# jjfiv/fastrank

Hardware: AMD Instinct MI355X
Metric: coordinate-ascent NDCG@10 evals/sec on MSLR-WEB30K shape (higher is better)
Workload: dtype f64; 1 GPU; synthetic MSLR-WEB30K shape: 3800000 docs x 136 features x 31000 queries, coordinate ascent NDCG@10, 32 restarts/GPU x 25 steps/coord (configs[2]); restarts_total=32, parallelism=restart-sharded x1 (dataset replicated), launcher=single process

## Files before the change

fastrank_amd/clib.py:

```python
import ctypes as C
import json
import os
from typing import Dict, List, Optional, Set

from . import _build

_MODEL_TYPES = ["SingleFeature", "Linear", "DecisionTree", "Ensemble"]


ALLREDUCE_SUM_FN = C.CFUNCTYPE(C.c_int, C.c_void_p, C.POINTER(C.c_double), C.c_size_t)


class _CResult(C.Structure):
    _fields_ = [("error_message", C.c_void_p), ("success", C.c_void_p)]


_lib = None


def _load():
    global _lib
    if _lib is not None:
        return _lib
    path = _build.LIB_PATH
    if _build.needs_build():
        try:
            _build.build()
        except Exception as exc:
            if not os.path.exists(path):
                raise ImportError(
                    "libfastrank_amd.so is not built and could not be built: {}".format(exc)
                ) from exc
    L = C.CDLL(path)
    vp, sz = C.c_void_p, C.c_size_t
    res = C.POINTER(_CResult)
    sigs = {
        "free_str": (None, [vp]),
        "free_c_result": (None, [res]),
        "free_dataset": (None, [vp]),
        "free_model": (None, [vp]),
        "free_cqrel": (None, [vp]),
        "load_cqrel": (res, [C.c_char_p]),
        "cqrel_from_json": (res, [C.c_char_p]),
        "cqrel_query_json": (vp, [vp, C.c_char_p]),
        "load_ranksvm_format": (res, [C.c_char_p, C.c_char_p]),
        "dataset_query_sampling": (res, [vp, C.c_char_p]),
        "dataset_feature_sampling": (res, [vp, C.c_char_p]),
        "dataset_query_json": (vp, [vp, C.c_char_p]),
        "query_json": (vp, [C.c_char_p]),
        "make_dense_dataset_f32_f64_i64": (res, [sz, sz, vp, vp, vp]),
        "train_model": (res, [C.c_char_p, vp]),
        "model_from_json": (res, [C.c_char_p]),
        "model_query_json": (vp, [vp, C.c_char_p]),
        "evaluate_by_query": (vp, [vp, vp, vp, C.c_char_p]),
        "predict_scores": (vp, [vp, vp]),
        "predict_to_trecrun": (vp, [vp, vp, C.c_char_p, C.c_char_p, sz]),
        "fr_device_count": (C.c_int, []),
        "fr_set_device": (C.c_int, [C.c_int]),
        "fr_version": (C.c_char_p, []),
        "fr_train_model_shard": (vp, [C.c_char_p, vp, C.c_uint32, C.c_uint32]),
        "fr_select_model": (res, [C.c_char_p, C.c_int]),
        "fr_ca_begin": (vp, [C.c_char_p, vp, C.c_uint32, C.c_uint32, C.POINTER(vp)]),
        "fr_ca_begin_query_shard": (vp, [C.c_char_p, vp, C.c_uint64, ALLREDUCE_SUM_FN, vp, C.POINTER(vp)]),
        "fr_ca_step": (vp, [vp, C.c_uint64, C.POINTER(C.c_uint64), C.POINTER(C.c_int)]),
        "fr_ca_state": (vp, [vp]),
        "fr_ca_free": (None, [vp]),
        "fr_last_train_stats": (vp, []),
        "fr_predict_scores_dense": (vp, [vp, vp, vp, sz]),
        "fr_debug_lambda_gradients": (vp, [vp, vp, vp, C.c_char_p, C.c_double, vp, vp, sz]),
        "fr_debug_hist_bins": (vp, [vp, C.c_uint32, sz, sz, vp, vp, vp, vp, vp]),
        "fr_debug_hist_tree": (res, [vp, C.c_uint32, C.c_uint32, C.c_uint32, vp, vp, sz]),
        "fr_debug_lambdamart_sample": (vp, [vp, C.c_char_p, C.c_uint32]),
        "fr_debug_lambda_gradients_sampled": (vp, [vp, vp, vp, C.c_char_p, C.c_double, vp, sz, vp, vp, sz]),
        "fr_debug_hist_tree_sampled": (res, [vp, C.c_uint32, C.c_uint32, C.c_uint32, vp, vp, sz, vp, sz, vp, sz]),
        "fr_evaluate_dense": (vp, [vp, vp, vp, C.c_char_p, vp, sz, C.POINTER(vp)]),
        "fr_rank_order": (vp, [vp, vp, vp, sz, vp, sz]),
        "fr_dataset_num_queries": (sz, [vp]),
        "fr_dataset_num_instances": (sz, [vp]),
        "fr_dataset_device_info": (vp, [vp]),
        "fr_evaluate_candidates": (vp, [vp, vp, C.c_char_p, sz, vp, vp, vp, vp, vp, vp]),
        "fr_profile_enable": (None, [C.c_int]),
        "fr_profile_reset": (None, []),
        "fr_profile_json": (vp, []),
        "fr_debug_resident_bound": (C.c_double, [C.c_int, C.c_double, C.c_double, C.c_double]),
        "fr_synchronize": (C.c_int, []),
        "fr_debug_device_plan": (vp, [C.c_char_p, C.c_int, C.c_uint32, C.c_int]),
        "fr_debug_fullrank_class": (C.c_uint32, [C.c_uint32]),
        "fr_debug_restart_queue": (vp, [C.c_uint32, C.c_uint32, C.c_uint32, vp, C.c_uint32]),
        "fr_dataset_release_replicas": (sz, [vp]),
        "fr_debug_peer_copy": (vp, [C.c_int, C.c_int, sz]),
        "fr_pack_restart_records": (vp, [C.c_char_p, sz, sz, vp]),
        "fr_unpack_restart_records": (vp, [vp, sz, sz]),
        "fr_rccl_allgather": (vp, [vp, sz, vp, sz, vp]),
        "fr_debug_rccl_selftest": (vp, [C.c_int]),
        "fr_debug_walk_tiles": (vp, [vp, vp, vp, sz, vp, vp, sz, sz]),
    }
    for name, (restype, argtypes) in sigs.items():
        fn = getattr(L, name)
        fn.restype = restype
        fn.argtypes = argtypes
    _lib = L
    return L


EXPORTED_SYMBOLS = None


def exported_symbols() -> List[str]:
    _load()
    return [
        "free_str", "free_c_result", "free_dataset", "free_model", "free_cqrel", "load_cqrel",
        "cqrel_from_json", "cqrel_query_json", "load_ranksvm_format", "dataset_query_sampling",
        "dataset_feature_sampling", "dataset_query_json", "query_json",
        "make_dense_dataset_f32_f64_i64", "train_model", "model_from_json", "model_query_json",
        "evaluate_by_query", "predict_scores", "predict_to_trecrun",
    ]


def _take_str(ptr) -> Optional[str]:
    if not ptr:
        return None
    try:
        return C.cast(ptr, C.c_char_p).value.decode("utf-8")
    finally:
        _load().free_str(ptr)


def _raise_if_error_str(text: Optional[str]):
    if text is None:
        return
    if "{" in text:
        payload = json.loads(text)
        if "error" in payload and "context" in payload:
            raise Exception("{0}: {1}".format(payload["error"], payload["context"]))
    else:
        raise Exception(text)


def _raise_if_error_json(payload):
    if isinstance(payload, dict) and "error" in payload and "context" in payload:
        raise Exception("{0}: {1}".format(payload["error"], payload["context"]))


def _unwrap(result_ptr):
    if not result_ptr:
        raise ValueError("CResult should not be NULL")
    res = result_ptr.contents
    err_ptr, ok_ptr = res.error_message, res.success
    _load().free_c_result(result_ptr)
    _raise_if_error_str(_take_str(err_ptr))
    return ok_ptr


def _status(ptr):
    _raise_if_error_str(_take_str(ptr))


def _json_reply(ptr):
    payload = json.loads(_take_str(ptr))
    _raise_if_error_json(payload)
    return payload


class CQRel:

    def __init__(self, pointer=None):
        self.pointer = pointer
        self._queries = None

    def __del__(self):
        if getattr(self, "pointer", None) is not None and _lib is not None:
            _lib.free_cqrel(self.pointer)
            self.pointer = None

    @staticmethod
    def load_file(path: str) -> "CQRel":
        return CQRel(_unwrap(_load().load_cqrel(path.encode("utf-8"))))

# ... 207 lines not shown
```

fastrank_amd/csrc/capi.cpp:

```cpp
#include <atomic>
#include <limits>
#include <chrono>
#include <cstdio>
#include <cstdlib>
#include <cstring>
#include <fstream>

#include "../../include/fastrank.h"
#include "host.hpp"
#include "loader.hpp"
#include "lambdamart.hpp"
#include "rf_train.hpp"

using fr::FrError;
using frjson::Value;

struct CDataset {
    std::shared_ptr<fr::DatasetView> view;
};
struct CModel {
    fr::Model actual;
};
struct CQRel {
    fr::QRel actual;
// ... 961 lines not shown

const void* fr_debug_peer_copy(int src_device, int dst_device, size_t bytes) {
    return json_call([&]() {
        int can = 0, en = 0;
        double ms = 0.0;
        std::string err;
        if (!frdev::peer_copy_probe(src_device, dst_device, bytes, &can, &en, &ms, &err)) fr::fail_str(err);
        Value o = Value::object();
        o.set("src", Value::uint((uint64_t)src_device));
        o.set("dst", Value::uint((uint64_t)dst_device));
        o.set("bytes", Value::uint((uint64_t)bytes));
        o.set("can_access", Value::boolean(can != 0));
        o.set("enabled", Value::boolean(en != 0));
        o.set("ms", Value::number(ms));
        o.set("gbps", Value::number(ms > 0.0 ? (double)bytes / (ms * 1e-3) / 1e9 : 0.0));
        return frjson::dump(o);
    });
}

static std::vector<fr::RestartResult> restarts_from_json_text(const std::string& text) {
    Value v = parse_json_or_fail(text);
    if (!v.is_array()) fr::fail_raw("Error(\"invalid type: expected a sequence\", line: 1, column: 1)");
    std::vector<fr::RestartResult> hist;
    for (const auto& r : v.arr) {
        fr::RestartResult h;
        h.restart_id = (uint32_t)fr::json_u64(fr::json_field(r, "restart_id"), "restart_id");
        h.score = fr::json_f64(fr::json_field(r, "score"), "score");
        for (const auto& x : fr::json_field(r, "weights").arr) h.weights.push_back(fr::json_f64(x, "weights"));
        hist.push_back(std::move(h));
    }
    return hist;
}

const void* fr_pack_restart_records(const void* restarts_json, size_t cap, size_t dim, double* out) {
    return status_call([&]() {
        if (out == nullptr) fr::fail_str("fr_pack_restart_records: null output buffer");
        fr::pack_restart_records(restarts_from_json_text(accept_str("restarts_json", restarts_json)), cap, dim, out);
    });
}

const void* fr_unpack_restart_records(const double* records, size_t n_records, size_t dim) {
    return json_call([&]() {
        if (records == nullptr && n_records > 0) fr::fail_str("fr_unpack_restart_records: null input buffer");
        return frjson::dump(restarts_to_json(fr::unpack_restart_records(records, n_records, dim)));
    });
}

const void* fr_rccl_allgather(const int* devices, size_t n, const double* blocks, size_t block_len, double* out) {
    return json_call([&]() {
        if ((devices == nullptr || blocks == nullptr) && n > 0) fr::fail_str("fr_rccl_allgather: null argument");
        std::vector<int> devs(devices, devices + n);
        frdev::RcclReport rep;
        std::vector<double> got;
        std::string err;
        if (!frdev::rccl_allgather(devs, blocks, block_len, &got, &rep, &err)) fr::fail_str(err);
        if (rep.ran && out != nullptr) std::memcpy(out, got.data(), got.size() * sizeof(double));
        return frjson::dump(rccl_report_to_json(rep));
    });
}

const void* fr_debug_walk_tiles(const uint32_t* run_pos, const uint32_t* run_q0, const uint32_t* run_q1, size_t nruns, const uint32_t* qstart,
                                const uint32_t* qlen, size_t nq, size_t np) {
    return json_call([&]() {
        if (nruns > 0 && (!run_pos || !run_q0 || !run_q1)) fr::fail_str("fr_debug_walk_tiles: null run table");
        if (nq > 0 && (!qstart || !qlen)) fr::fail_str("fr_debug_walk_tiles: null query table");
        for (size_t q = 0; q < nq; q++)
            if ((size_t)qstart[q] + qlen[q] > np) fr::fail_str("fr_debug_walk_tiles: a query lies beyond np");
        for (size_t r = 0; r < nruns; r++)
            if (run_q0[r] > run_q1[r] || run_q1[r] > nq) fr::fail_str("fr_debug_walk_tiles: a run names queries that do not exist");
        const frdev::WalkTileLayout wl = frdev::build_walk_tiles(std::vector<uint32_t>(run_pos, run_pos + nruns), std::vector<uint32_t>(run_q0, run_q0 + nruns),
                                                                std::vector<uint32_t>(run_q1, run_q1 + nruns), std::vector<uint32_t>(qstart, qstart + nq),
                                                                std::vector<uint32_t>(qlen, qlen + nq), np);
        Value o = Value::object();
        auto list = [](const auto& v) {
            Value a = Value::array();
            for (auto x : v) a.push(Value::uint((uint64_t)x));
            return a;
        };
        o.set("walk_tile", Value::uint(frdev::WALK_TILE));
        o.set("wt_start", list(wl.wt_start));
        o.set("run_wt0", list(wl.run_wt0));
        o.set("seg", list(wl.seg));
        o.set("wofs", list(wl.wofs));
        return frjson::dump(o);
    });
}

const void* fr_debug_rccl_selftest(int device) {
    return json_call([&]() {
        std::vector<double> block(16), got;
        for (size_t i = 0; i < block.size(); i++) block[i] = 0.5 + (double)i;
        frdev::RcclReport rep;
        std::string err;
        if (!frdev::rccl_allgather(std::vector<int>(1, device), block.data(), block.size(), &got, &rep, &err, 1)) fr::fail_str(err);
        return frjson::dump(rccl_report_to_json(rep));
    });
}

int fr_set_device(int ordinal) {
    std::string err;
    if (!frdev::set_device(ordinal, &err)) return 1;
    frdev::warm_device(ordinal);
    g_pinned_device = ordinal;
    return 0;
}

const char* fr_version(void) { return "fastrank_amd 0.1.0 (fastrank C ABI 0.9.0-dev / python 0.7.0)"; }

const void* fr_train_model_shard(const void* train_request_json, const CDataset* dataset, uint32_t restart_begin,
                                 uint32_t restart_end) {
    return json_call([&]() {
        const CDataset& ds = require_dataset(dataset);
        ParsedRequest rq = parse_train_request(accept_str("train_request_json", train_request_json));
        if (rq.learner != Learner::CoordinateAscent) fr::fail_str("fr_train_model_shard: only CoordinateAscent shards by restart");
        std::lock_guard<std::mutex> lk(api_mu_of(ds));
        std::vector<fr::RestartResult> hist;
        train_ca(ds.view, rq, restart_begin, restart_end, &hist);
        Value o = Value::object();
        o.set("restarts", restarts_to_json(hist));
        {
            std::lock_guard<std::mutex> slk(g_stats_mu);
            o.set("stats", stats_to_json(g_last_stats));
        }
        return frjson::dump(o);
    });
}

struct FrTrainer {
    std::unique_ptr<fr::CATrainer> t;
    std::chrono::steady_clock::time_point t0;
    std::shared_ptr<fr::DataCore> core;
};

void* fr_ca_begin(const void* train_request_json, const CDataset* dataset, uint32_t restart_begin,
                  uint32_t restart_end, const void** error_out) {
    if (error_out) *error_out = nullptr;
    FrTrainer* h = nullptr;
    const void* st = status_call([&]() {
        const CDataset& ds = require_dataset(dataset);
        ParsedRequest rq = parse_train_request(accept_str("train_request_json", train_request_json));
        if (rq.learner != Learner::CoordinateAscent) fr::fail_str("fr_ca_begin: only CoordinateAscent");
        std::lock_guard<std::mutex> lk(api_mu_of(ds));
        fr::Evaluator ev = fr::make_evaluator(*ds.view, rq.measure, rq.has_qrel ? &rq.qrel : nullptr);
        if (ds.view->host_csr().nq == 0) fr::fail_str("assertion failed: !data.queries().is_empty()");
        auto holder = std::make_unique<FrTrainer>();
        holder->t0 = std::chrono::steady_clock::now();
        holder->t = std::make_unique<fr::CATrainer>(ds.view, std::move(ev), rq.ca, restart_begin, restart_end);
        holder->core = ds.view->core;
        h = holder.release();
    });
    if (st) {
        if (error_out) *error_out = st; else free((void*)st);
        return nullptr;
    }
    return h;
}

void* fr_ca_begin_query_shard(const void* train_request_json, const CDataset* dataset, uint64_t total_queries,
                              fr_allreduce_sum_fn allreduce, void* ctx, const void** error_out) {
    if (error_out) *error_out = nullptr;
    FrTrainer* h = nullptr;
    const void* st = status_call([&]() {
        const CDataset& ds = require_dataset(dataset);
        ParsedRequest rq = parse_train_request(accept_str("train_request_json", train_request_json));
        if (rq.learner != Learner::CoordinateAscent) fr::fail_str("fr_ca_begin_query_shard: only CoordinateAscent");
        if (!allreduce) fr::fail_str("fr_ca_begin_query_shard: allreduce callback is null!");
// ... 458 lines not shown
```

fastrank_amd/csrc/device.hpp:

```cpp
#pragma once
#include <algorithm>
#include <cstddef>
#include <cstdint>
#include <memory>
#include <string>
#include <vector>

namespace frdev {

const char* path_env(const char* name);
inline const char* pricing_env(const char* name) {
#ifdef FR_PRICING
    return path_env(name);
#else
    (void)name;
    return nullptr;
#endif
}

enum Measure : int { M_NDCG = 0, M_AP = 1, M_RR = 2 };

constexpr uint32_t WALK_TILE = 128;
struct WalkTileLayout {
    std::vector<uint32_t> wt_start, run_wt0;
// ... 134 lines not shown
        unsigned long long pairs = 0, redone = 0;
    };
    bool linesearch_submit(int ctx, int measure, int64_t depth, const double* norms, const std::vector<LineGroup>& groups,
                           std::string* err);
    bool linesearch_collect(int ctx, std::vector<double>* means, LsCounts* counts, std::string* err);
    bool linesearch(int measure, int64_t depth, const double* norms, const std::vector<LineGroup>& groups,
                    std::vector<double>* means, LsCounts* counts, std::string* err);
    uint64_t resident_reserve(size_t slots, std::string* err);
    bool resident_store_from_scores(uint64_t owner, size_t slot, size_t b, std::string* err);
    const std::vector<double>& column_absmax() const;
    unsigned long long exact_fallbacks() const;
    void routing_counters(unsigned long long* exact_groups, unsigned long long* redo_entries) const;
    void chain_counters(unsigned long long* runs, unsigned long long* visits, unsigned long long* ranked_on = nullptr,
                        unsigned long long* ranked_off = nullptr) const;
    void audit_counters(unsigned long long* values, unsigned long long* mismatches) const;
    bool download_last_matrix(std::vector<double>* out, size_t* ldm, std::string* err);

    struct RfActive { uint32_t tree, key, n; };
    struct RfCand { double position, importance; uint32_t ids_i, flags, pos_l, pos_r; double sum_l, sum_r; };
    struct RfSplit { int32_t fslot; uint32_t pos, left, right; };
    bool rf_set_presence(const uint32_t* bits_by_instance, size_t words, size_t n_instances, std::string* err);
    bool rf_begin(const std::vector<uint32_t>& root_off, const std::vector<uint32_t>& root_ids, uint32_t nf,
                  const std::vector<uint32_t>& feats, std::string* err, const uint32_t* positions = nullptr,
                  bool lambda_targets = false);
    bool rf_positions(const std::vector<uint32_t>& root_ids, uint32_t* positions , std::string* err);
    bool rf_root_outputs(std::vector<double>* out, std::string* err);
    bool rf_level(const std::vector<RfActive>& active, const std::vector<uint32_t>& slot_of_key, uint32_t k, int method,
                  uint32_t min_leaf, std::vector<RfCand>* cands, std::vector<float>* label_minmax, std::string* err);
    bool rf_split(const std::vector<RfSplit>& splits, std::vector<double>* child_out, std::string* err);
    void rf_end();
    size_t rf_bytes_per_item() const { return 41; }

    bool lambda_gradients(const double* norms, int64_t depth, double sigma, std::string* err, const unsigned char* query_flags = nullptr);
    bool lambda_download_positions(std::vector<double>* lambda, std::vector<double>* weight, std::string* err);
    bool lambda_download(double* lambda_by_instance, double* weight_by_instance, size_t out_len, std::string* err,
                         const unsigned char* query_flags = nullptr);

    struct HistNode { uint32_t slot, begin, end; };
    struct HistSplit { uint32_t begin, end, fslot, edge, nl; };
    struct HistSub { uint32_t parent, small, large; };
    struct HistBest { double imp; long long ql, qtot; uint32_t edge, nl, valid, pad; };
    bool hist_bins(const uint32_t* positions, size_t n, const std::vector<uint32_t>& feats, uint32_t k, bool* built, std::string* err);
    bool hist_edges(std::vector<float>* edges, std::vector<uint32_t>* nedges, std::string* err);
    bool hist_download_bins(uint8_t* out , size_t len, std::string* err);
    bool hist_sample(const unsigned char* query_flags, uint32_t n_t, const uint32_t* fsel, size_t f_t, std::string* err);
    bool hist_quantise(const double* lam_list, const double* wt_list, int* s_l, int* s_w, bool* all_zero, std::string* err);
    bool hist_root(std::string* err);
    bool hist_search(const std::vector<HistNode>& nodes, uint32_t min_leaf, std::vector<HistBest>* best, std::string* err);
    bool hist_split(const std::vector<HistSplit>& splits, const std::vector<HistNode>& builds, const std::vector<HistSub>& subs,
                    uint32_t next_slots, std::string* err);
    bool hist_leaf_sums(const std::vector<HistNode>& leaves, std::vector<long long>* qw , std::string* err);
    void hist_end();

    int take_flags();

  private:
    DeviceDataset();
    bool try_score_trees_rank(const FlatTrees& trees, std::string* err);
    bool try_score_trees_lds(const FlatTrees& trees, std::string* err);
    bool try_score_trees_lds_shape(const FlatTrees& trees, const void* shape, std::string* err);
    struct Impl;
    Impl* impl_;
};

int device_count(std::string* err);
bool set_device(int ordinal, std::string* err);
void warm_device(int ordinal);
void profile_enable(bool on);
void profile_reset();
std::vector<KernelStat> profile_stats();
bool device_synchronize(std::string* err);
struct RcclReport {
    bool ran = false, matches_host_gather = false;
    int ranks = 0;
    std::vector<int> devices;
    size_t block_doubles = 0;
    double init_us = 0.0, first_us = 0.0, us = 0.0;
    std::string reason;
    std::string library;
};
bool rccl_allgather(const std::vector<int>& devices, const double* blocks, size_t block_len, std::vector<double>* gathered, RcclReport* rep,
                    std::string* err, size_t min_ranks = 2);
bool peer_copy_probe(int src, int dst, size_t bytes, int* can_access, int* enabled, double* ms, std::string* err);
size_t device_free_bytes();
void* pinned_alloc(size_t bytes);
void pinned_free(void* p);
void fullrank_class_of(uint32_t len, uint32_t* nl, uint32_t* pl);

}
```

fastrank_amd/csrc/kernels_order.inc:

```
constexpr uint32_t WT = WALK_TILE;
constexpr uint32_t WT_DPL = WT / 64;

__device__ __forceinline__ void order_segment(uint32_t s, uint32_t idx, uint32_t len, uint32_t* lo, uint32_t* hi) {
    *lo = s & 0xFFu;
    *hi = s >> 8;
    if (idx >= len || *hi <= *lo) {
        *lo = idx;
        *hi = idx + 1u;
    }
}

constexpr int ORDER_OQ = 2;
__global__ __launch_bounds__(WAVE) void xslot_kernel(const float4* __restrict__ xb, const uint16_t* __restrict__ seg, const uint32_t* __restrict__ wt_start,
                                                     uint32_t np, uint32_t dq, uint32_t d, uint8_t* __restrict__ out) {
    __shared__ float4 xs[ORDER_OQ][WT];
    const uint32_t lane = threadIdx.x;
    const uint32_t pb = wt_start[blockIdx.x];
    const uint32_t len = min(wt_start[blockIdx.x + 1] - pb, WT);
    const uint32_t j0 = blockIdx.y * ORDER_OQ;
    uint32_t lo[WT_DPL], hi[WT_DPL];
    float4 mine[WT_DPL][ORDER_OQ];
#pragma unroll
    for (uint32_t h = 0; h < WT_DPL; h++) {
        const uint32_t idx = lane + 64u * h;
        const uint32_t p = pb + (idx < len ? idx : 0u);
        order_segment(seg[p], idx, len, &lo[h], &hi[h]);
#pragma unroll
        for (int u = 0; u < ORDER_OQ; u++) {
            const uint32_t j4 = j0 + u < dq ? j0 + u : dq - 1;
            const float4 v = xb[((size_t)(p >> 6) * dq + j4) * 64 + (p & 63u)];
            const float ninf = -__builtin_huge_valf();
            mine[h][u] = make_float4(v.x == v.x ? v.x : ninf, v.y == v.y ? v.y : ninf, v.z == v.z ? v.z : ninf, v.w == v.w ? v.w : ninf);
            xs[u][idx] = mine[h][u];
        }
    }
    __syncthreads();
#pragma unroll
    for (uint32_t h = 0; h < WT_DPL; h++) {
        const uint32_t idx = lane + 64u * h;
        if (idx >= len) continue;
        uint32_t r[ORDER_OQ][4];
#pragma unroll
        for (int u = 0; u < ORDER_OQ; u++)
#pragma unroll
            for (int k = 0; k < 4; k++) r[u][k] = 0;
        for (uint32_t i = lo[h]; i < hi[h]; i++) {
            const bool before = i < idx;
#pragma unroll
            for (int u = 0; u < ORDER_OQ; u++) {
                const float4 o = xs[u][i];
                r[u][0] += (o.x > mine[h][u].x) || (o.x == mine[h][u].x && before);
                r[u][1] += (o.y > mine[h][u].y) || (o.y == mine[h][u].y && before);
                r[u][2] += (o.z > mine[h][u].z) || (o.z == mine[h][u].z && before);
                r[u][3] += (o.w > mine[h][u].w) || (o.w == mine[h][u].w && before);
            }
        }
#pragma unroll
        for (int u = 0; u < ORDER_OQ; u++)
#pragma unroll
            for (int k = 0; k < 4; k++) {
                const uint32_t f = (j0 + u) * 4 + k;
                if (j0 + u < dq && f < d) out[(size_t)f * np + pb + idx] = (uint8_t)(lo[h] + r[u][k]);
            }
    }
}

__global__ __launch_bounds__(WAVE) void xcol_kernel(const float4* __restrict__ xb, uint32_t np, uint32_t dq, uint32_t d, float* __restrict__ out) {
    const uint32_t lane = threadIdx.x, tile = blockIdx.x;
    const size_t p = (size_t)tile * 64u + lane;
    const uint32_t j0 = blockIdx.y * ORDER_OQ;
    float4 v[ORDER_OQ];
#pragma unroll
    for (int u = 0; u < ORDER_OQ; u++) v[u] = xb[((size_t)tile * dq + (j0 + u < dq ? j0 + u : dq - 1)) * 64 + lane];
#pragma unroll
    for (int u = 0; u < ORDER_OQ; u++) {
        const uint32_t f = (j0 + u) * 4;
        if (j0 + u < dq) {
            if (f + 0 < d) out[(size_t)(f + 0) * np + p] = v[u].x;
            if (f + 1 < d) out[(size_t)(f + 1) * np + p] = v[u].y;
            if (f + 2 < d) out[(size_t)(f + 2) * np + p] = v[u].z;
            if (f + 3 < d) out[(size_t)(f + 3) * np + p] = v[u].w;
        }
    }
}

template <uint32_t J, uint32_t KK, uint32_t HI>
__device__ __forceinline__ uint32_t order_exchange(uint32_t key, uint32_t lane) {
    constexpr uint64_t keep_min = [] {
        uint64_t m = 0;
        for (uint32_t l = 0; l < 64; l++) {
            const uint32_t e = l + 64u * HI;
            const bool up = (e & KK) == 0u, lower = (e & J) == 0u;
            if (up == lower) m |= 1ull << l;
        }
        return m;
    }();
    const uint32_t other = (uint32_t)__builtin_amdgcn_ds_bpermute((int)((lane ^ J) << 2), (int)key);
    const uint32_t mn = key < other ? key : other, mx = key < other ? other : key;
    return ((keep_min >> lane) & 1ull) ? mn : mx;
}
template <uint32_t KK, uint32_t HI>
__device__ __forceinline__ uint32_t order_merge(uint32_t key, uint32_t lane) {
    if constexpr (KK >= 64) key = order_exchange<32, KK, HI>(key, lane);
    if constexpr (KK >= 32) key = order_exchange<16, KK, HI>(key, lane);
    if constexpr (KK >= 16) key = order_exchange<8, KK, HI>(key, lane);
    if constexpr (KK >= 8) key = order_exchange<4, KK, HI>(key, lane);
    if constexpr (KK >= 4) key = order_exchange<2, KK, HI>(key, lane);
    return order_exchange<1, KK, HI>(key, lane);
}
static_assert(WT == 128, "the sort below is the 128-element network (two registers per lane)");
constexpr uint32_t RSLOT_BATCH = 4;
__global__ __launch_bounds__(256) void rslot_kernel(const double* __restrict__ res, const int32_t* __restrict__ slot_half,
                                                     const int32_t* __restrict__ slot_group, uint32_t nlist, const double* __restrict__ rs_par,
                                                     const uint32_t* __restrict__ rs_updf, const float* __restrict__ xcol,
                                                     const uint16_t* __restrict__ seg, const uint32_t* __restrict__ wt_start,
                                                     const uint32_t* __restrict__ wlist, uint32_t nw, uint32_t np, uint8_t* __restrict__ out) {
    const uint32_t lane = threadIdx.x & 63u, wi = blockIdx.x * 4u + (threadIdx.x >> 6);
    if (wi >= nw) return;
    const uint32_t ti = wlist ? wlist[wi] : wi;
    const uint32_t pb = wt_start[ti];
    const uint32_t len = min(wt_start[ti + 1] - pb, WT);
    uint32_t p[2], sidx[2];
    {
        uint32_t lo0, hi0, lo1, hi1;
        p[0] = pb + (lane < len ? lane : 0u);
        p[1] = pb + (lane + 64u < len ? lane + 64u : 0u);
        order_segment(seg[p[0]], lane, len, &lo0, &hi0);
        order_segment(seg[p[1]], lane + 64u, len, &lo1, &hi1);
        const uint64_t s0 = __ballot(lo0 == lane), s1 = __ballot(lo1 == lane + 64u);
        const uint64_t upto = (lane >= 63u) ? ~0ull : ((2ull << lane) - 1ull);
        sidx[0] = (uint32_t)__popcll(s0 & upto) - 1u;
        sidx[1] = (uint32_t)__popcll(s0) + (uint32_t)__popcll(s1 & upto) - 1u;
    }
    for (uint32_t k0 = 0; k0 < nlist; k0 += RSLOT_BATCH) {
        float r[RSLOT_BATCH][2];
        int32_t sh[RSLOT_BATCH];
#pragma unroll
        for (uint32_t u = 0; u < RSLOT_BATCH; u++) {
            const uint32_t k = k0 + u < nlist ? k0 + u : nlist - 1;
            sh[u] = slot_half[k];
            double R0 = res[(size_t)sh[u] * np + p[0]], R1 = res[(size_t)sh[u] * np + p[1]];
            const double* par = rs_par + (size_t)slot_group[k] * 6;
            if (par[2] != 0.0) {
                const float* xu = xcol + (size_t)rs_updf[slot_group[k]] * np;
                const double x0 = (double)xu[p[0]], x1 = (double)xu[p[1]];
                R0 = __builtin_fma(x0, par[5], __builtin_fma(-x0, par[4], R0 * par[3]));
                R1 = __builtin_fma(x1, par[5], __builtin_fma(-x1, par[4], R1 * par[3]));
            }
            r[u][0] = (float)R0;
            r[u][1] = (float)R1;
        }
#pragma unroll
        for (uint32_t u = 0; u < RSLOT_BATCH; u++) {
            if (k0 + u >= nlist) break;
            uint32_t key[2];
#pragma unroll
            for (uint32_t h = 0; h < 2; h++) {
                const uint32_t bits = __float_as_uint(r[u][h] == r[u][h] ? r[u][h] : -__builtin_huge_valf());
                const uint32_t mono = bits ^ ((uint32_t)((int32_t)bits >> 31) | 0x80000000u);
                key[h] = (sidx[h] << 25) | ((~mono >> 14) << 7) | (lane + 64u * h);
            }
            key[0] = order_merge<2, 0>(key[0], lane), key[1] = order_merge<2, 1>(key[1], lane);
            key[0] = order_merge<4, 0>(key[0], lane), key[1] = order_merge<4, 1>(key[1], lane);
            key[0] = order_merge<8, 0>(key[0], lane), key[1] = order_merge<8, 1>(key[1], lane);
            key[0] = order_merge<16, 0>(key[0], lane), key[1] = order_merge<16, 1>(key[1], lane);
            key[0] = order_merge<32, 0>(key[0], lane), key[1] = order_merge<32, 1>(key[1], lane);
            key[0] = order_merge<64, 0>(key[0], lane), key[1] = order_merge<64, 1>(key[1], lane);
            {
                const uint32_t mn = key[0] < key[1] ? key[0] : key[1], mx = key[0] < key[1] ? key[1] : key[0];
                key[0] = mn, key[1] = mx;
            }
            key[0] = order_merge<64, 0>(key[0], lane);
            key[1] = order_merge<64, 0>(key[1], lane);
#pragma unroll
            for (uint32_t h = 0; h < 2; h++) {
                const uint32_t from = key[h] & 127u;
                if (from < len) out[(size_t)(sh[u] >> 1) * np + pb + from] = (uint8_t)(lane + 64u * h);
            }
        }
    }
}

__global__ void rslot_identity_kernel(uint8_t* __restrict__ out, const uint8_t* __restrict__ wofs, size_t np, size_t n) {
    for (size_t i = (size_t)blockIdx.x * blockDim.x + threadIdx.x; i < n; i += (size_t)gridDim.x * blockDim.x) out[i] = wofs[i % np];
}

__global__ __launch_bounds__(256) void order_audit_kernel(const uint8_t* __restrict__ table, const uint16_t* __restrict__ seg,
                                                           const uint32_t* __restrict__ wt_start, const uint32_t* __restrict__ wlist, uint32_t nw,
                                                           unsigned long long* bad) {
    __shared__ uint32_t hits[4][WT];
    const uint32_t lane = threadIdx.x & 63u, w = threadIdx.x >> 6, wi = blockIdx.x * 4u + w;
    const bool on = wi < nw;
    const uint32_t ti = on ? (wlist ? wlist[wi] : wi) : 0u;
    const uint32_t pb = wt_start[ti];
    const uint32_t len = on ? min(wt_start[ti + 1] - pb, WT) : 0u;
    for (uint32_t h = 0; h < WT_DPL; h++) hits[w][lane + 64u * h] = 0u;
    __syncthreads();
    unsigned long long mine = 0;
    for (uint32_t h = 0; h < WT_DPL; h++) {
        const uint32_t idx = lane + 64u * h;
        if (idx >= len) continue;
        const uint16_t s = seg[pb + idx];
        const uint32_t lo = s & 0xFFu, hi = s >> 8;
        if (hi <= lo) continue;
        const uint32_t slot = table[pb + idx];
        if (slot < lo || slot >= hi) mine++;
        else atomicAdd(&hits[w][slot], 1u);
    }
    __syncthreads();
    for (uint32_t h = 0; h < WT_DPL; h++) {
        const uint32_t idx = lane + 64u * h;
        if (idx >= len) continue;
        const uint16_t s = seg[pb + idx];
        if ((s >> 8) > (s & 0xFFu) && hits[w][idx] != 1u) mine++;
    }
    if (mine) atomicAdd(bad, mine);
}

struct ColStats {
    double sum, sumsq;
    float mn, mx;
    unsigned long long at_min, at_max;
};
__global__ __launch_bounds__(256) void colstats_kernel(const float4* __restrict__ xb, const uint16_t* __restrict__ seg, uint32_t ntiles, uint32_t dq,
                                                       uint32_t d, int pass, ColStats* __restrict__ st) {
    const uint32_t lane = threadIdx.x & 63u, w = threadIdx.x >> 6, j4 = blockIdx.y;
    double s[4] = {0, 0, 0, 0}, s2[4] = {0, 0, 0, 0};
    float mn[4], mx[4];
    unsigned long long cmin[4] = {0, 0, 0, 0}, cmax[4] = {0, 0, 0, 0};
    float emin[4], emax[4];
#pragma unroll
    for (int k = 0; k < 4; k++) {
        mn[k] = __builtin_huge_valf();
        mx[k] = -__builtin_huge_valf();
        const uint32_t f = j4 * 4 + k;
        emin[k] = (pass == 1 && f < d) ? st[f].mn : 0.0f;
        emax[k] = (pass == 1 && f < d) ? st[f].mx : 0.0f;
    }
    for (uint32_t t = blockIdx.x * 4 + w; t < ntiles; t += gridDim.x * 4) {
        const uint16_t sg = seg[(size_t)t * 64 + lane];
        if ((sg >> 8) <= (sg & 0xFF)) continue;
        const float4 v = xb[((size_t)t * dq + j4) * 64 + lane];
        const float x[4] = {v.x, v.y, v.z, v.w};
#pragma unroll
        for (int k = 0; k < 4; k++) {
            if (pass == 0) {
                s[k] += (double)x[k];
                s2[k] += (double)x[k] * (double)x[k];
                mn[k] = x[k] < mn[k] ? x[k] : mn[k];
                mx[k] = x[k] > mx[k] ? x[k] : mx[k];
            } else {
                cmin[k] += x[k] == emin[k];
                cmax[k] += x[k] == emax[k];
            }
        }
    }
#pragma unroll
    for (int k = 0; k < 4; k++) {
        const uint32_t f = j4 * 4 + k;
        if (f >= d) continue;
        if (pass == 0) {
            atomicAdd(&st[f].sum, s[k]);
            atomicAdd(&st[f].sumsq, s2[k]);
            if (mn[k] >= 0.0f) atomicMin(reinterpret_cast<int*>(&st[f].mn), __float_as_int(mn[k]));
            else atomicMax(reinterpret_cast<unsigned int*>(&st[f].mn), __float_as_uint(mn[k]));
            if (mx[k] >= 0.0f) atomicMax(reinterpret_cast<int*>(&st[f].mx), __float_as_int(mx[k]));
            else atomicMin(reinterpret_cast<unsigned int*>(&st[f].mx), __float_as_uint(mx[k]));
        } else {
            if (cmin[k]) atomicAdd(&st[f].at_min, cmin[k]);
            if (cmax[k]) atomicAdd(&st[f].at_max, cmax[k]);
        }
    }
}
```

fastrank_amd/native.py:

```python
import ctypes as C
import json
from typing import Dict, List, Optional, Tuple

import numpy as np

from .clib import ALLREDUCE_SUM_FN, CDataset, CModel, CQRel, _json_reply, _load, _status, _take_str, _unwrap


def device_count() -> int:
    return int(_load().fr_device_count())


def set_device(ordinal: int) -> None:
    if _load().fr_set_device(int(ordinal)) != 0:
        raise RuntimeError("fr_set_device({}) failed".format(ordinal))


def version() -> str:
    return _load().fr_version().decode("utf-8")


def synchronize() -> None:
    if _load().fr_synchronize() != 0:
        raise RuntimeError("device synchronize failed")
# ... 229 lines not shown
        def reduce_cb(_ctx, values, n):
            try:
                arr = np.ctypeslib.as_array(values, shape=(n,))
                arr[:] = rank_ordered_sum(arr, group)
                return 0
            except Exception as exc:
                self._callback_error = exc
                return 1

        self._callback_error = None
        self._callback = ALLREDUCE_SUM_FN(reduce_cb)
        err = C.c_void_p()
        request = json.dumps(train_req.to_dict()).encode("utf-8")
        self.pointer = _load().fr_ca_begin_query_shard(request, dataset.pointer, int(total_queries), self._callback, None, C.byref(err))
        if not self.pointer:
            _status(err.value)
            raise RuntimeError("fr_ca_begin_query_shard failed")
        self._dataset = dataset
        self.finished = False
        self.total_queries = int(total_queries)


def train_model_query_sharded(dataset: CDataset, train_req, total_queries: Optional[int] = None, group=None) -> CModel:
    run = QueryShardedRun(dataset, train_req, total_queries, group)
    try:
        while not run.finished:
            run.step(1 << 20)
        restarts = run.state()["restarts"]
    finally:
        run.close()
    model = select_model(restarts, bool(train_req.params.output_ensemble))
    model.params = train_req
    return model


def select_model(restarts: List[Dict], output_ensemble: bool = False) -> CModel:
    payload = json.dumps(restarts).encode("utf-8")
    return CModel(_unwrap(_load().fr_select_model(payload, 1 if output_ensemble else 0)))


def device_plan(devices: str, device_count: int, num_restarts: int, primary_device: int = 0) -> Dict:
    return _json_reply(_load().fr_debug_device_plan(devices.encode("utf-8"), device_count, num_restarts, primary_device))


def restart_queue_replay(num_restarts: int, n_workers: int, capacity: int, lengths) -> Dict:
    arr = np.ascontiguousarray(lengths, dtype=np.uint32)
    return _json_reply(_load().fr_debug_restart_queue(int(num_restarts), int(n_workers), int(capacity), arr.ctypes.data, len(arr)))


def peer_copy(src_device: int, dst_device: int, nbytes: int = 256 << 20) -> Dict:
    return _json_reply(_load().fr_debug_peer_copy(int(src_device), int(dst_device), int(nbytes)))


def pack_restart_records(restarts: List[Dict], cap: int, dim: int) -> "np.ndarray":
    out = np.zeros((int(cap), 3 + int(dim)), dtype=np.float64)
    _status(_load().fr_pack_restart_records(json.dumps(restarts).encode("utf-8"), int(cap), int(dim), out.ctypes.data))
    return out


def unpack_restart_records(records: "np.ndarray", dim: int) -> List[Dict]:
    arr = np.ascontiguousarray(records, dtype=np.float64).reshape(-1, 3 + int(dim))
    return _json_reply(_load().fr_unpack_restart_records(arr.ctypes.data, arr.shape[0], int(dim)))


def rccl_allgather_restarts(devices: List[int], parts: List[List[Dict]]) -> Tuple[Dict, Optional[List[Dict]]]:
    n = len(devices)
    cap = max([1] + [len(p) for p in parts])
    dim = max([0] + [len(r["weights"]) for p in parts for r in p])
    blocks = np.stack([pack_restart_records(p, cap, dim) for p in parts]) if n else np.zeros((0, cap, 3 + dim))
    out = np.empty_like(blocks)
    devs = np.ascontiguousarray(devices, dtype=np.int32)
    rep = _json_reply(_load().fr_rccl_allgather(devs.ctypes.data, n, blocks.ctypes.data, cap * (3 + dim), out.ctypes.data))
    if not rep.get("ran"):
        return rep, None
    if not np.array_equal(out.view(np.uint64), blocks.view(np.uint64)):
        raise RuntimeError("rccl_allgather_restarts: rank 0's gathered records differ from the blocks the ranks contributed")
    return rep, unpack_restart_records(out, dim)


def walk_tiles(run_pos, run_q0, run_q1, qstart, qlen, np_positions: int) -> Dict:
    arrs = [np.ascontiguousarray(a, dtype=np.uint32) for a in (run_pos, run_q0, run_q1, qstart, qlen)]
    return _json_reply(_load().fr_debug_walk_tiles(arrs[0].ctypes.data, arrs[1].ctypes.data, arrs[2].ctypes.data, len(arrs[0]),
                                                   arrs[3].ctypes.data, arrs[4].ctypes.data, len(arrs[3]), int(np_positions)))


def rccl_selftest(device: int = 0) -> Dict:
    return _json_reply(_load().fr_debug_rccl_selftest(int(device)))


def release_replicas(dataset: CDataset) -> int:
    return int(_load().fr_dataset_release_replicas(dataset.pointer))


def shard_bounds(num_restarts: int, rank: int, world: int) -> Tuple[int, int]:
    base, rem = divmod(num_restarts, world)
    begin = rank * base + min(rank, rem)
    return begin, begin + base + (1 if rank < rem else 0)


def gather_restarts(mine: List[Dict], num_restarts: int, group=None) -> List[Dict]:
    import torch
    import torch.distributed as dist

    if not dist.is_available() or not dist.is_initialized():
        return sorted(mine, key=lambda r: r["restart_id"])
    world = dist.get_world_size(group)
    backend = dist.get_backend(group)
    dev = torch.device("cuda", torch.cuda.current_device()) if backend == "nccl" else torch.device("cpu")
    shape_t = torch.tensor([max((len(r["weights"]) for r in mine), default=0), len(mine)], dtype=torch.int64, device=dev)
    dist.all_reduce(shape_t, op=dist.ReduceOp.MAX, group=group)
    dim, per_rank = int(shape_t[0].item()), max(1, int(shape_t[1].item()))
    buf = torch.zeros((per_rank, 3 + dim), dtype=torch.float64)
    for k, r in enumerate(mine):
        buf[k, 0] = 1.0
        buf[k, 1] = float(r["restart_id"])
        buf[k, 2] = r["score"]
        buf[k, 3:3 + len(r["weights"])] = torch.tensor(r["weights"], dtype=torch.float64)
    buf = buf.to(dev)
    gathered = [torch.empty_like(buf) for _ in range(world)]
    dist.all_gather(gathered, buf, group=group)
    restarts = []
    for t in gathered:
        for row in t.cpu().tolist():
            if row[0] == 1.0:
                restarts.append({"restart_id": int(row[1]), "score": row[2], "weights": row[3:]})
    restarts.sort(key=lambda r: r["restart_id"])
    if len(restarts) != num_restarts or any(r["restart_id"] != i for i, r in enumerate(restarts)):
        raise RuntimeError("gather_restarts: expected restarts 0..{} exactly once, got {}".format(
            num_restarts - 1, [r["restart_id"] for r in restarts]))
    return restarts


_steal_jobs = 0


def steal_blocks(num_restarts: int, block: int, group=None, store=None):
    import torch.distributed as dist

    global _steal_jobs
    key = "fastrank_amd/steal/{}".format(_steal_jobs)
    _steal_jobs += 1
    if not dist.is_available() or not dist.is_initialized():
        for b in range(0, num_restarts, block):
            yield b, min(num_restarts, b + block)
        return
    if store is None:
        store = dist.distributed_c10d._get_default_store()
    while True:
        k = int(store.add(key, 1)) - 1
        if k * block >= num_restarts:
            return
        yield k * block, min(num_restarts, (k + 1) * block)


def train_model_work_stealing(dataset: CDataset, train_req, block: int = 8, group=None, store=None, stats: Optional[Dict] = None) -> CModel:
    R = int(train_req.params.num_restarts)
    mine, blocks = [], []
    for begin, end in steal_blocks(R, block, group, store):
        shard = train_model_shard(dataset, train_req, begin, end)
        mine.extend(shard["restarts"])
        blocks.append((begin, end))
    if stats is not None:
        stats["blocks"] = blocks
    restarts = gather_restarts(mine, R, group)
    model = select_model(restarts, bool(train_req.params.output_ensemble))
    model.params = train_req
# ... 17 lines not shown
```

include/fastrank.h:

```cpp
#ifndef FASTRANK_AMD_H
#define FASTRANK_AMD_H

#include <stddef.h>
#include <stdint.h>

#ifdef __cplusplus
extern "C" {
#endif

typedef struct CDataset CDataset;
typedef struct CModel CModel;
typedef struct CQRel CQRel;

typedef struct CResult {
    const void *error_message;
    const void *success;
} CResult;


void free_str(void *originally_from_library);
void free_c_result(CResult *originally_from_library);
void free_dataset(CDataset *originally_from_library);
void free_model(CModel *originally_from_library);
void free_cqrel(CQRel *originally_from_library);
// ... 8 lines not shown
const void *dataset_query_json(void *dataset, void *json_cmd_str);
const void *query_json(const void *json_cmd_str);

const CResult *make_dense_dataset_f32_f64_i64(size_t n, size_t d, const float *x, const double *y,
                                              const int64_t *qids);

const CResult *train_model(void *train_request_json, void *dataset);
const CResult *model_from_json(const void *json_str);
const void *model_query_json(const void *model, const void *json_cmd_str);

const void *evaluate_by_query(const CModel *model, const CDataset *dataset, const CQRel *qrel,
                              const void *evaluator_name);
const void *predict_scores(const CModel *model, const CDataset *dataset);
const void *predict_to_trecrun(const CModel *model, const CDataset *dataset, const void *output_path,
                               const void *system_name, size_t depth);


int fr_device_count(void);
int fr_set_device(int ordinal);
const char *fr_version(void);

const void *fr_train_model_shard(const void *train_request_json, const CDataset *dataset,
                                 uint32_t restart_begin, uint32_t restart_end);
void *fr_ca_begin(const void *train_request_json, const CDataset *dataset, uint32_t restart_begin,
                  uint32_t restart_end, const void **error_out);
typedef int (*fr_allreduce_sum_fn)(void *ctx, double *values, size_t n);
void *fr_ca_begin_query_shard(const void *train_request_json, const CDataset *dataset, uint64_t total_queries,
                              fr_allreduce_sum_fn allreduce, void *ctx, const void **error_out);
const void *fr_ca_step(void *trainer, uint64_t max_ticks, uint64_t *ticks_done, int *finished);
const void *fr_ca_state(void *trainer);
void fr_ca_free(void *trainer);

const CResult *fr_select_model(const void *restarts_json, int output_ensemble);
const void *fr_last_train_stats(void);

const void *fr_predict_scores_dense(const CModel *model, const CDataset *dataset, double *out, size_t out_len);
const void *fr_evaluate_dense(const CModel *model, const CDataset *dataset, const CQRel *qrel,
                              const void *evaluator_name, double *out_values, size_t out_len,
                              const void **out_qids_json);
const void *fr_debug_lambda_gradients(const CModel *model, const CDataset *dataset, const CQRel *qrel,
                                      const void *measure, double sigma, double *lambda_out,
                                      double *weight_out, size_t out_len);
const void *fr_debug_hist_bins(const CDataset *dataset, uint32_t split_candidates, size_t n, size_t f,
                               uint32_t *ids_out, uint32_t *feats_out, float *edges_out,
                               uint32_t *nedges_out, uint8_t *bins_out);
const CResult *fr_debug_hist_tree(const CDataset *dataset, uint32_t split_candidates, uint32_t max_depth,
                                  uint32_t min_leaf_support, const double *lambda, const double *weight,
                                  size_t len);
const void *fr_debug_lambdamart_sample(const CDataset *dataset, const void *params_json, uint32_t tree);
const void *fr_debug_lambda_gradients_sampled(const CModel *model, const CDataset *dataset, const CQRel *qrel,
                                              const void *measure, double sigma, const uint32_t *queries,
                                              size_t n_queries, double *lambda_out, double *weight_out,
                                              size_t out_len);
const CResult *fr_debug_hist_tree_sampled(const CDataset *dataset, uint32_t split_candidates, uint32_t max_depth,
                                          uint32_t min_leaf_support, const double *lambda, const double *weight,
                                          size_t len, const uint32_t *queries, size_t n_queries,
                                          const uint32_t *features, size_t n_features);
const void *fr_rank_order(const CModel *model, const CDataset *dataset, uint32_t *out_instance_ids,
                          size_t n, uint64_t *out_offsets, size_t nq_plus_1);
const void *fr_dataset_device_info(const CDataset *dataset);
size_t fr_dataset_num_queries(const CDataset *dataset);
size_t fr_dataset_num_instances(const CDataset *dataset);

const void *fr_evaluate_candidates(const CDataset *dataset, const CQRel *qrel, const void *evaluator_name,
                                   size_t n_groups, const uint32_t *features, const double *base_weights,
                                   const uint32_t *n_cand, const double *candidates, double *out_means,
                                   double *out_per_query);

void fr_profile_enable(int on);
void fr_profile_reset(void);
const void *fr_profile_json(void);
int fr_synchronize(void);
double fr_debug_resident_bound(int which, double a, double b, double c);
uint32_t fr_debug_fullrank_class(uint32_t len);
const void *fr_debug_device_plan(const void *devices_csv, int device_count, uint32_t num_restarts, int primary_device);
const void *fr_debug_restart_queue(uint32_t num_restarts, uint32_t n_workers, uint32_t capacity, const uint32_t *lengths,
                                   uint32_t n_lengths);
const void *fr_debug_peer_copy(int src_device, int dst_device, size_t bytes);
const void *fr_pack_restart_records(const void *restarts_json, size_t cap, size_t dim, double *out);
const void *fr_unpack_restart_records(const double *records, size_t n_records, size_t dim);
const void *fr_rccl_allgather(const int *devices, size_t n, const double *blocks, size_t block_len, double *out);
const void *fr_debug_walk_tiles(const uint32_t *run_pos, const uint32_t *run_q0, const uint32_t *run_q1, size_t nruns,
                                const uint32_t *qstart, const uint32_t *qlen, size_t nq, size_t np);
const void *fr_debug_rccl_selftest(int device);
size_t fr_dataset_release_replicas(const CDataset *dataset);

#ifdef __cplusplus
}
#endif
#endif
```

Before: 716,700 evals/s.

## Replace bpermute bitonic sort in rslot kernel with DPP/permlane swap network

Rewrites the 128-element per-wave bitonic sort used in the rslot kernel. LDS-based ds_bpermute exchanges are replaced by a remapped lane/element bit layout that uses register-local compare-exchanges, DPP row/quad ops and v_permlane16/32_swap instructions. Direction flips are applied by XOR masks computed once per wave instead of per-stage keep_min masks. The aim is lower latency and less LDS traffic per sort. It adds inline assembly that depends on the gfx950 ISA, and the output slot index has to be remapped. A debug probe entry point is also added to check the resulting table.

```diff
diff --git a/fastrank_amd/clib.py b/fastrank_amd/clib.py
--- a/fastrank_amd/clib.py
+++ b/fastrank_amd/clib.py
@@ -94,6 +94,7 @@
         "fr_rccl_allgather": (vp, [vp, sz, vp, sz, vp]),
         "fr_debug_rccl_selftest": (vp, [C.c_int]),
         "fr_debug_walk_tiles": (vp, [vp, vp, vp, sz, vp, vp, sz, sz]),
+        "fr_debug_rslot": (vp, [vp, vp, vp, vp, vp, sz, vp, sz, sz, vp]),
     }
     for name, (restype, argtypes) in sigs.items():
         fn = getattr(L, name)
diff --git a/fastrank_amd/csrc/capi.cpp b/fastrank_amd/csrc/capi.cpp
--- a/fastrank_amd/csrc/capi.cpp
+++ b/fastrank_amd/csrc/capi.cpp
@@ -1067,6 +1067,18 @@
         o.set("run_wt0", list(wl.run_wt0));
         o.set("seg", list(wl.seg));
         o.set("wofs", list(wl.wofs));
+        return frjson::dump(o);
+    });
+}
+
+const void* fr_debug_rslot(const double* sums, const float* xupd, const double* par6, const uint16_t* seg, const uint32_t* wt_start, size_t ntiles,
+                           const uint32_t* wlist, size_t nw, size_t np, uint8_t* table) {
+    return json_call([&]() {
+        unsigned long long bad = 0;
+        std::string err;
+        if (!frdev::rslot_probe(sums, xupd, par6, seg, wt_start, ntiles, wlist, nw, np, table, &bad, &err)) fr::fail_str(err);
+        Value o = Value::object();
+        o.set("audit_bad", Value::uint((uint64_t)bad));
         return frjson::dump(o);
     });
 }
diff --git a/fastrank_amd/csrc/device.hpp b/fastrank_amd/csrc/device.hpp
--- a/fastrank_amd/csrc/device.hpp
+++ b/fastrank_amd/csrc/device.hpp
@@ -240,6 +240,8 @@
 bool rccl_allgather(const std::vector<int>& devices, const double* blocks, size_t block_len, std::vector<double>* gathered, RcclReport* rep,
                     std::string* err, size_t min_ranks = 2);
 bool peer_copy_probe(int src, int dst, size_t bytes, int* can_access, int* enabled, double* ms, std::string* err);
+bool rslot_probe(const double* sums, const float* xupd, const double* par6, const uint16_t* seg, const uint32_t* wt_start, size_t ntiles,
+                 const uint32_t* wlist, size_t nw, size_t np, uint8_t* table, unsigned long long* bad, std::string* err);
 size_t device_free_bytes();
 void* pinned_alloc(size_t bytes);
 void pinned_free(void* p);
diff --git a/fastrank_amd/csrc/kernels_order.inc b/fastrank_amd/csrc/kernels_order.inc
--- a/fastrank_amd/csrc/kernels_order.inc
+++ b/fastrank_amd/csrc/kernels_order.inc
@@ -84,29 +84,90 @@
     }
 }
 
-template <uint32_t J, uint32_t KK, uint32_t HI>
-__device__ __forceinline__ uint32_t order_exchange(uint32_t key, uint32_t lane) {
-    constexpr uint64_t keep_min = [] {
-        uint64_t m = 0;
-        for (uint32_t l = 0; l < 64; l++) {
-            const uint32_t e = l + 64u * HI;
-            const bool up = (e & KK) == 0u, lower = (e & J) == 0u;
-            if (up == lower) m |= 1ull << l;
-        }
-        return m;
-    }();
-    const uint32_t other = (uint32_t)__builtin_amdgcn_ds_bpermute((int)((lane ^ J) << 2), (int)key);
-    const uint32_t mn = key < other ? key : other, mx = key < other ? other : key;
-    return ((keep_min >> lane) & 1ull) ? mn : mx;
-}
-template <uint32_t KK, uint32_t HI>
-__device__ __forceinline__ uint32_t order_merge(uint32_t key, uint32_t lane) {
-    if constexpr (KK >= 64) key = order_exchange<32, KK, HI>(key, lane);
-    if constexpr (KK >= 32) key = order_exchange<16, KK, HI>(key, lane);
-    if constexpr (KK >= 16) key = order_exchange<8, KK, HI>(key, lane);
-    if constexpr (KK >= 8) key = order_exchange<4, KK, HI>(key, lane);
-    if constexpr (KK >= 4) key = order_exchange<2, KK, HI>(key, lane);
-    return order_exchange<1, KK, HI>(key, lane);
+constexpr uint32_t RS_LANE_BIT[7] = {0, 3, 4, 5, 2, 1, 0};
+__device__ __forceinline__ uint32_t rs_element(uint32_t lane) {
+    uint32_t e = 0;
+#pragma unroll
+    for (uint32_t b = 1; b < 7; b++) e |= ((lane >> RS_LANE_BIT[b]) & 1u) << b;
+    return e;
+}
+__device__ __forceinline__ uint32_t rs_bitmask(uint32_t lane, uint32_t b) { return b < 7 ? 0u - ((lane >> RS_LANE_BIT[b]) & 1u) : 0u; }
+__device__ __forceinline__ void rs_cx_reg(uint32_t& k0, uint32_t& k1) {
+    const uint32_t mn = k0 < k1 ? k0 : k1, mx = k0 < k1 ? k1 : k0;
+    k0 = mn, k1 = mx;
+}
+__device__ __forceinline__ void rs_cx_swap16(uint32_t& k0, uint32_t& k1) {
+    uint32_t t;
+    asm volatile("s_nop 1\n\tv_permlane16_swap_b32 %0, %1\n\ts_nop 1\n\tv_min_u32 %2, %0, %1\n\tv_max_u32 %1, %0, %1\n\ts_nop 1\n\t"
+                 "v_permlane16_swap_b32 %2, %1"
+                 : "+v"(k0), "+v"(k1), "=&v"(t));
+    k0 = t;
+}
+__device__ __forceinline__ void rs_cx_swap32(uint32_t& k0, uint32_t& k1) {
+    uint32_t t;
+    asm volatile("s_nop 1\n\tv_permlane32_swap_b32 %0, %1\n\ts_nop 1\n\tv_min_u32 %2, %0, %1\n\tv_max_u32 %1, %0, %1\n\ts_nop 1\n\t"
+                 "v_permlane32_swap_b32 %2, %1"
+                 : "+v"(k0), "+v"(k1), "=&v"(t));
+    k0 = t;
+}
+__device__ __forceinline__ void rs_cx_lane3(uint32_t& k0, uint32_t& k1) {
+    uint32_t t0, t1;
+    asm volatile("s_nop 1\n\t"
+                 "v_min_u32_dpp %0, %2, %2 row_ror:8 row_mask:0xf bank_mask:0x3\n\t"
+                 "v_min_u32_dpp %1, %3, %3 row_ror:8 row_mask:0xf bank_mask:0x3\n\t"
+                 "v_max_u32_dpp %0, %2, %2 row_ror:8 row_mask:0xf bank_mask:0xc\n\t"
+                 "v_max_u32_dpp %1, %3, %3 row_ror:8 row_mask:0xf bank_mask:0xc"
+                 : "=&v"(t0), "=&v"(t1)
+                 : "v"(k0), "v"(k1));
+    k0 = t0, k1 = t1;
+}
+__device__ __forceinline__ void rs_cx_lane2(uint32_t& k0, uint32_t& k1) {
+    uint32_t t0, t1;
+    asm volatile("s_nop 1\n\t"
+                 "v_min_u32_dpp %0, %2, %2 row_shl:4 row_mask:0xf bank_mask:0x5\n\t"
+                 "v_min_u32_dpp %1, %3, %3 row_shl:4 row_mask:0xf bank_mask:0x5\n\t"
+                 "v_max_u32_dpp %0, %2, %2 row_shr:4 row_mask:0xf bank_mask:0xa\n\t"
+                 "v_max_u32_dpp %1, %3, %3 row_shr:4 row_mask:0xf bank_mask:0xa"
+                 : "=&v"(t0), "=&v"(t1)
+                 : "v"(k0), "v"(k1));
+    k0 = t0, k1 = t1;
+}
+#define RS_CX_QUAD(NAME, PERM)                                                                                          \
+    __device__ __forceinline__ void NAME(uint32_t& k0, uint32_t& k1, uint64_t odd) {                                    \
+        uint32_t a0, a1, b0, b1;                                                                                        \
+        asm volatile("s_nop 1\n\t"                                                                                      \
+                     "v_min_u32_dpp %0, %4, %4 quad_perm:" PERM " row_mask:0xf bank_mask:0xf\n\t"                        \
+                     "v_min_u32_dpp %1, %5, %5 quad_perm:" PERM " row_mask:0xf bank_mask:0xf\n\t"                        \
+                     "v_max_u32_dpp %2, %4, %4 quad_perm:" PERM " row_mask:0xf bank_mask:0xf\n\t"                        \
+                     "v_max_u32_dpp %3, %5, %5 quad_perm:" PERM " row_mask:0xf bank_mask:0xf\n\t"                        \
+                     "v_cndmask_b32_e64 %0, %0, %2, %6\n\t"                                                             \
+                     "v_cndmask_b32_e64 %1, %1, %3, %6"                                                                 \
+                     : "=&v"(a0), "=&v"(a1), "=&v"(b0), "=&v"(b1)                                                       \
+                     : "v"(k0), "v"(k1), "s"(odd));                                                                     \
+        k0 = a0, k1 = a1;                                                                                               \
+    }
+RS_CX_QUAD(rs_cx_lane1, "[2,3,0,1]")
+RS_CX_QUAD(rs_cx_lane0, "[1,0,3,2]")
+#undef RS_CX_QUAD
+template <uint32_t B>
+__device__ __forceinline__ void rs_cx(uint32_t& k0, uint32_t& k1, uint64_t odd1, uint64_t odd0) {
+    if constexpr (B == 0) rs_cx_reg(k0, k1);
+    else if constexpr (B == 1) rs_cx_lane3(k0, k1);
+    else if constexpr (B == 2) rs_cx_swap16(k0, k1);
+    else if constexpr (B == 3) rs_cx_swap32(k0, k1);
+    else if constexpr (B == 4) rs_cx_lane2(k0, k1);
+    else if constexpr (B == 5) rs_cx_lane1(k0, k1, odd1);
+    else rs_cx_lane0(k0, k1, odd0);
+}
+template <uint32_t KB>
+__device__ __forceinline__ void rs_merge(uint32_t& k0, uint32_t& k1, uint64_t odd1, uint64_t odd0) {
+    if constexpr (KB >= 7) rs_cx<6>(k0, k1, odd1, odd0);
+    if constexpr (KB >= 6) rs_cx<5>(k0, k1, odd1, odd0);
+    if constexpr (KB >= 5) rs_cx<4>(k0, k1, odd1, odd0);
+    if constexpr (KB >= 4) rs_cx<3>(k0, k1, odd1, odd0);
+    if constexpr (KB >= 3) rs_cx<2>(k0, k1, odd1, odd0);
+    if constexpr (KB >= 2) rs_cx<1>(k0, k1, odd1, odd0);
+    rs_cx<0>(k0, k1, odd1, odd0);
 }
 static_assert(WT == 128, "the sort below is the 128-element network (two registers per lane)");
 constexpr uint32_t RSLOT_BATCH = 4;
@@ -132,6 +193,12 @@
         sidx[0] = (uint32_t)__popcll(s0 & upto) - 1u;
         sidx[1] = (uint32_t)__popcll(s0) + (uint32_t)__popcll(s1 & upto) - 1u;
     }
+    uint32_t flip[7];
+    flip[0] = rs_bitmask(lane, 1);
+#pragma unroll
+    for (uint32_t i = 1; i < 7; i++) flip[i] = rs_bitmask(lane, i) ^ rs_bitmask(lane, i + 1);
+    const uint64_t odd1 = __ballot((lane & 2u) != 0u), odd0 = __ballot((lane & 1u) != 0u);
+    const uint32_t elem = rs_element(lane);
     for (uint32_t k0 = 0; k0 < nlist; k0 += RSLOT_BATCH) {
         float r[RSLOT_BATCH][2];
         int32_t sh[RSLOT_BATCH];
@@ -160,22 +227,24 @@
                 const uint32_t mono = bits ^ ((uint32_t)((int32_t)bits >> 31) | 0x80000000u);
                 key[h] = (sidx[h] << 25) | ((~mono >> 14) << 7) | (lane + 64u * h);
             }
-            key[0] = order_merge<2, 0>(key[0], lane), key[1] = order_merge<2, 1>(key[1], lane);
-            key[0] = order_merge<4, 0>(key[0], lane), key[1] = order_merge<4, 1>(key[1], lane);
-            key[0] = order_merge<8, 0>(key[0], lane), key[1] = order_merge<8, 1>(key[1], lane);
-            key[0] = order_merge<16, 0>(key[0], lane), key[1] = order_merge<16, 1>(key[1], lane);
-            key[0] = order_merge<32, 0>(key[0], lane), key[1] = order_merge<32, 1>(key[1], lane);
-            key[0] = order_merge<64, 0>(key[0], lane), key[1] = order_merge<64, 1>(key[1], lane);
-            {
-                const uint32_t mn = key[0] < key[1] ? key[0] : key[1], mx = key[0] < key[1] ? key[1] : key[0];
-                key[0] = mn, key[1] = mx;
-            }
-            key[0] = order_merge<64, 0>(key[0], lane);
-            key[1] = order_merge<64, 0>(key[1], lane);
+            key[0] ^= flip[0], key[1] ^= flip[0];
+            rs_merge<1>(key[0], key[1], odd1, odd0);
+            key[0] ^= flip[1], key[1] ^= flip[1];
+            rs_merge<2>(key[0], key[1], odd1, odd0);
+            key[0] ^= flip[2], key[1] ^= flip[2];
+            rs_merge<3>(key[0], key[1], odd1, odd0);
+            key[0] ^= flip[3], key[1] ^= flip[3];
+            rs_merge<4>(key[0], key[1], odd1, odd0);
+            key[0] ^= flip[4], key[1] ^= flip[4];
+            rs_merge<5>(key[0], key[1], odd1, odd0);
+            key[0] ^= flip[5], key[1] ^= flip[5];
+            rs_merge<6>(key[0], key[1], odd1, odd0);
+            key[0] ^= flip[6], key[1] ^= flip[6];
+            rs_merge<7>(key[0], key[1], odd1, odd0);
 #pragma unroll
             for (uint32_t h = 0; h < 2; h++) {
                 const uint32_t from = key[h] & 127u;
-                if (from < len) out[(size_t)(sh[u] >> 1) * np + pb + from] = (uint8_t)(lane + 64u * h);
+                if (from < len) out[(size_t)(sh[u] >> 1) * np + pb + from] = (uint8_t)(elem | h);
             }
         }
     }
@@ -217,6 +286,64 @@
     if (mine) atomicAdd(bad, mine);
 }
 
+bool rslot_probe(const double* sums, const float* xupd, const double* par6, const uint16_t* seg, const uint32_t* wt_start, size_t ntiles,
+                 const uint32_t* wlist, size_t nw, size_t np, uint8_t* table, unsigned long long* bad, std::string* err) {
+    if (!sums || !xupd || !par6 || !seg || !wt_start || !table || !bad || np == 0 || np >= (size_t(1) << 31)) {
+        if (err) *err = "rslot_probe: null or empty argument";
+        return false;
+    }
+    if (!wlist) nw = ntiles;
+    for (size_t i = 0; i < nw; i++) {
+        const size_t ti = wlist ? wlist[i] : i;
+        if (ti >= ntiles || wt_start[ti] >= np || wt_start[ti + 1] < wt_start[ti] ||
+            (size_t)wt_start[ti] + std::min<size_t>(wt_start[ti + 1] - wt_start[ti], WT) > np) {
+            if (err) *err = "rslot_probe: a listed walk tile lies outside the positions";
+            return false;
+        }
+    }
+    for (size_t p = 0; p < np; p++)
+        if ((seg[p] & 0xFFu) > WT || (seg[p] >> 8) > WT) {
+            if (err) *err = "rslot_probe: a segment reaches beyond its walk tile";
+            return false;
+        }
+    if (nw == 0) {
+        std::memset(table, 0xFF, np);
+        *bad = 0;
+        return true;
+    }
+    DevBuf<double> d_res, d_par;
+    DevBuf<float> d_x;
+    DevBuf<uint16_t> d_seg;
+    DevBuf<uint32_t> d_wt, d_wl, d_updf;
+    DevBuf<int32_t> d_list;
+    DevBuf<uint8_t> d_out;
+    DevBuf<unsigned long long> d_bad;
+    if (!d_res.ensure(np, err) || !d_par.ensure(6, err) || !d_x.ensure(np, err) || !d_seg.ensure(np, err) || !d_wt.ensure(ntiles + 1, err) ||
+        !d_wl.ensure(std::max<size_t>(nw, 1), err) || !d_updf.ensure(1, err) || !d_list.ensure(2, err) || !d_out.ensure(np, err) || !d_bad.ensure(1, err))
+        return false;
+    const int32_t list[2] = {0, 0};
+    const uint32_t updf = 0;
+    FR_HIP(hipMemcpy(d_res.p, sums, np * sizeof(double), hipMemcpyHostToDevice));
+    FR_HIP(hipMemcpy(d_par.p, par6, 6 * sizeof(double), hipMemcpyHostToDevice));
+    FR_HIP(hipMemcpy(d_x.p, xupd, np * sizeof(float), hipMemcpyHostToDevice));
+    FR_HIP(hipMemcpy(d_seg.p, seg, np * sizeof(uint16_t), hipMemcpyHostToDevice));
+    FR_HIP(hipMemcpy(d_wt.p, wt_start, (ntiles + 1) * sizeof(uint32_t), hipMemcpyHostToDevice));
+    if (wlist) FR_HIP(hipMemcpy(d_wl.p, wlist, nw * sizeof(uint32_t), hipMemcpyHostToDevice));
+    FR_HIP(hipMemcpy(d_updf.p, &updf, sizeof(updf), hipMemcpyHostToDevice));
+    FR_HIP(hipMemcpy(d_list.p, list, sizeof(list), hipMemcpyHostToDevice));
+    FR_HIP(hipMemset(d_out.p, 0xFF, np));
+    FR_HIP(hipMemset(d_bad.p, 0, sizeof(unsigned long long)));
+    const uint32_t* wl = wlist ? d_wl.p : nullptr;
+    rslot_kernel<<<dim3((unsigned)((nw + 3) / 4)), 256>>>(d_res.p, d_list.p, d_list.p + 1, 1u, d_par.p, d_updf.p, d_x.p, d_seg.p, d_wt.p, wl, (uint32_t)nw,
+                                                          (uint32_t)np, d_out.p);
+    FR_HIP(hipGetLastError());
+    order_audit_kernel<<<dim3((unsigned)((nw + 3) / 4)), 256>>>(d_out.p, d_seg.p, d_wt.p, wl, (uint32_t)nw, d_bad.p);
+    FR_HIP(hipGetLastError());
+    FR_HIP(hipMemcpy(table, d_out.p, np, hipMemcpyDeviceToHost));
+    FR_HIP(hipMemcpy(bad, d_bad.p, sizeof(unsigned long long), hipMemcpyDeviceToHost));
+    return true;
+}
+
 struct ColStats {
     double sum, sumsq;
     float mn, mx;
diff --git a/fastrank_amd/native.py b/fastrank_amd/native.py
--- a/fastrank_amd/native.py
+++ b/fastrank_amd/native.py
@@ -335,6 +335,23 @@
     arrs = [np.ascontiguousarray(a, dtype=np.uint32) for a in (run_pos, run_q0, run_q1, qstart, qlen)]
     return _json_reply(_load().fr_debug_walk_tiles(arrs[0].ctypes.data, arrs[1].ctypes.data, arrs[2].ctypes.data, len(arrs[0]),
                                                    arrs[3].ctypes.data, arrs[4].ctypes.data, len(arrs[3]), int(np_positions)))
+
+
+def rslot_table(sums, xupd, par6, seg, wt_start, np_positions: int, wlist=None) -> Tuple["np.ndarray", int]:
+    n = int(np_positions)
+    a_sums = np.ascontiguousarray(sums, dtype=np.float64)
+    a_x = np.ascontiguousarray(xupd, dtype=np.float32)
+    a_par = np.ascontiguousarray(par6, dtype=np.float64)
+    a_seg = np.ascontiguousarray(seg, dtype=np.uint16)
+    a_wt = np.ascontiguousarray(wt_start, dtype=np.uint32)
+    a_wl = None if wlist is None else np.ascontiguousarray(wlist, dtype=np.uint32)
+    if len(a_sums) != n or len(a_x) != n or len(a_seg) != n or len(a_par) != 6 or len(a_wt) < 1:
+        raise ValueError("rslot_table: array lengths do not match np_positions")
+    table = np.empty(n, dtype=np.uint8)
+    rep = _json_reply(_load().fr_debug_rslot(a_sums.ctypes.data, a_x.ctypes.data, a_par.ctypes.data, a_seg.ctypes.data, a_wt.ctypes.data,
+                                             len(a_wt) - 1, None if a_wl is None else a_wl.ctypes.data, 0 if a_wl is None else len(a_wl),
+                                             n, table.ctypes.data))
+    return table, int(rep["audit_bad"])
 
 
 def rccl_selftest(device: int = 0) -> Dict:
diff --git a/include/fastrank.h b/include/fastrank.h
--- a/include/fastrank.h
+++ b/include/fastrank.h
@@ -114,6 +114,8 @@
 const void *fr_rccl_allgather(const int *devices, size_t n, const double *blocks, size_t block_len, double *out);
 const void *fr_debug_walk_tiles(const uint32_t *run_pos, const uint32_t *run_q0, const uint32_t *run_q1, size_t nruns,
                                 const uint32_t *qstart, const uint32_t *qlen, size_t nq, size_t np);
+const void *fr_debug_rslot(const double *sums, const float *xupd, const double *par6, const uint16_t *seg, const uint32_t *wt_start,
+                           size_t ntiles, const uint32_t *wlist, size_t nw, size_t np, uint8_t *table);
 const void *fr_debug_rccl_selftest(int device);
 size_t fr_dataset_release_replicas(const CDataset *dataset);
 
```

Result: no change. 723,800 evals/s, median of 6 (+1.0%).
